# kenziyuliu/ChineseCheckersAgent

Hardware: AMD Instinct MI355X
Metric: mcts_node_expansions_per_s (self-play with the policy/value net, 4096 games x 400 sims/move per GPU); BASELINE games/s = config.games_per_s: selfplay() calls that RETURNED per second, discarded ones included (train.py:61-64 counts them); config.games_won_per_s: those that returned a history (higher is better)
Workload: dtype f32

## Files before the change

### chinesecheckersagent_amd/csrc/ccsp_net.hip

```cpp
#include <cmath>
#include <cstring>
#include <type_traits>
#include <vector>
#include "ccsp_common.h"

namespace {

typedef float f32x4 __attribute__((ext_vector_type(4)));

#ifndef CCSP_NET_LDX
#define CCSP_NET_LDX 68
#define CCSP_NET_LDY 36
#endif
constexpr int LDX = CCSP_NET_LDX;
constexpr int LDY = CCSP_NET_LDY;
constexpr int LDI = 12;
constexpr int NPOL = 294, NPOL_PAD = 304;
#ifndef CCSP_NET_LDS_BIAS_ALL
#define CCSP_NET_LDS_BIAS_ALL 0
#endif
#ifndef CCSP_NET_PDG
#define CCSP_NET_PDG 1
#endif
#ifndef CCSP_NET_SEG_STEM
#define CCSP_NET_SEG_STEM 1
#endif
#ifndef CCSP_NET_SEG_L1
#define CCSP_NET_SEG_L1 1
#endif
#ifndef CCSP_NET_SEG_L2
#define CCSP_NET_SEG_L2 4
#endif
#ifndef CCSP_NET_SEG_L3
#define CCSP_NET_SEG_L3 1
#endif
#ifndef CCSP_NET_SEG_PC
#define CCSP_NET_SEG_PC 1
#endif

struct Layout {
    int trunk_b;
    int stem_w, stem_b;
    int l1_w[9], l1_b[9], l2_w[9], l2_b[9], l3_w[9], l3_b[9];
    int pc_w, pc_b, pf_w, pf_b;
    int vc_w, vc_b, f1_w, f1_b, f2_w, f2_b;
    int total;
};

constexpr Layout make_layout() {
    Layout L{};
    int o = 0;
    auto take = [&](int n) { int r = o; o += (n + 3) & ~3; return r; };
    L.trunk_b = take(64 + 9 * 128 + 16);
    L.stem_w = take(4 * 5 * 256); L.stem_b = L.trunk_b;
    for (int i = 0; i < 9; i++) {
        L.l1_w[i] = take(2 * 4 * 256); L.l1_b[i] = L.trunk_b + 64 + i * 128;
        L.l2_w[i] = take(2 * 18 * 256); L.l2_b[i] = L.trunk_b + 64 + i * 128 + 32;
        L.l3_w[i] = take(4 * 2 * 256); L.l3_b[i] = L.trunk_b + 64 + i * 128 + 64;
    }
    L.pc_w = take(1 * 4 * 256); L.pc_b = L.trunk_b + 64 + 9 * 128;
    L.pf_w = take(5 * 100 * 256); L.pf_b = take(NPOL_PAD);
    L.vc_w = take(64); L.vc_b = take(1);
    L.f1_w = take(25 * 32); L.f1_b = take(32);
    L.f2_w = take(32); L.f2_b = take(1);
    L.total = o;
    return L;
}
constexpr Layout LAY = make_layout();
constexpr int BLK_STRIDE = LAY.l1_w[1] - LAY.l1_w[0];
constexpr bool layout_is_regular() {
    for (int i = 0; i < 9; i++)
        if (LAY.l1_w[i] != LAY.l1_w[0] + i * BLK_STRIDE || LAY.l2_w[i] != LAY.l2_w[0] + i * BLK_STRIDE || LAY.l3_w[i] != LAY.l3_w[0] + i * BLK_STRIDE) return false;
    return true;
}
static_assert(layout_is_regular(), "the blocks' weights are BLK_STRIDE floats apart");
constexpr int BIAS_STEM = 0, BIAS_BLK = 64, BIAS_PER_BLK = 128, BIAS_L1 = 0, BIAS_L2 = 32, BIAS_L3 = 64, BIAS_PC = BIAS_BLK + 9 * BIAS_PER_BLK, BIAS_N = BIAS_PC + 16;
static_assert(LAY.stem_b == LAY.trunk_b + BIAS_STEM && LAY.l1_b[3] == LAY.trunk_b + BIAS_BLK + 3 * BIAS_PER_BLK + BIAS_L1 && LAY.l2_b[8] == LAY.trunk_b + BIAS_BLK + 8 * BIAS_PER_BLK + BIAS_L2 &&
              LAY.l3_b[0] == LAY.trunk_b + BIAS_BLK + BIAS_L3 && LAY.pc_b == LAY.trunk_b + BIAS_PC && BIAS_N % 4 == 0 && LAY.trunk_b % 4 == 0, "Smem::bias is the blob's trunk_b region");

constexpr int PLAIN_TOTAL = 4032 + 64 + 9 * (2048 + 32 + 9216 + 32 + 2048 + 64) + 1024 + 16 + 117600 + 294 + 64 + 1 + 800 + 32 + 32 + 1;
static_assert(PLAIN_TOTAL == 244920, "249852 parameters minus the 4 x 1233 BatchNorm values folded away");

constexpr int PAD0 = 7, PADPOS = 36;
#ifndef CCSP_NET_SKIP_DEAD_TAPS
#define CCSP_NET_SKIP_DEAD_TAPS 1
#endif
#ifndef CCSP_NET_KB_FENCE
#define CCSP_NET_KB_FENCE 1
#endif
#ifndef CCSP_NET_CM4
#define CCSP_NET_CM4 1
#endif
constexpr unsigned char CELL8[25] = {0, 1, 2, 3, 6, 7,   4, 9, 14, 19, 11, 12,   24, 23, 22, 21, 16, 17,   20, 15, 10, 5, 8, 13,   18};
constexpr unsigned char CELL4[25] = {0, 1, 2, 3,  4, 9, 14, 19,  6, 7, 8, 11,   24, 23, 22, 21,  20, 15, 10, 5,  12, 13, 16, 17,   18};
constexpr int on_edge(int cell, int e) { return e == 0 ? cell / 5 == 0 : (e == 1 ? cell % 5 == 4 : (e == 2 ? cell / 5 == 4 : cell % 5 == 0)); }
constexpr bool interior(int cell) { return !on_edge(cell, 0) && !on_edge(cell, 1) && !on_edge(cell, 2) && !on_edge(cell, 3); }
constexpr bool cells_ok() {
    bool seen8[25] = {}, seen4[25] = {};
    for (int i = 0; i < 25; i++) {
        if (CELL8[i] > 24 || seen8[CELL8[i]] || CELL4[i] > 24 || seen4[CELL4[i]]) return false;
        seen8[CELL8[i]] = true; seen4[CELL4[i]] = true;
    }
    for (int g = 0; g < 4; g++)
        for (int i = 0; i < 6; i++)
            if (i < 4 ? !on_edge(CELL8[6 * g + i], g) : !interior(CELL8[6 * g + i])) return false;
    for (int g = 0; g < 2; g++)
        for (int i = 0; i < 12; i++)
            if (i < 8 ? !on_edge(CELL4[12 * g + i], 2 * g + i / 4) : !interior(CELL4[12 * g + i])) return false;
    return interior(CELL8[24]) && interior(CELL4[24]);
}
static_assert(cells_ok(), "CELL8 / CELL4: permutations; the edge tiles on their edges, the other tiles interior");
template <int NB>
constexpr unsigned long long cell_pack(int from) {
    unsigned long long v = 0;
    for (int i = 0; i < 12 && from + i < 25; i++) v |= (unsigned long long)(NB == 8 ? CELL8 : CELL4)[from + i] << (5 * i);
    return v;
}
template <int NB>
__device__ __forceinline__ int cell_of(int idx) {
    const unsigned long long w = idx < 12 ? cell_pack<NB>(0) : (idx < 24 ? cell_pack<NB>(12) : cell_pack<NB>(24));
    return (int)((w >> (5 * (idx < 12 ? idx : (idx < 24 ? idx - 12 : 0)))) & 31);
}
constexpr unsigned EDGE_DEAD[4] = {0x0003Fu , 0x30C30u , 0x3F000u , 0x030C3u };
constexpr int CM_PAD = 3, CM_SLOTS = 35;

template <int NBv, int NWv>
struct Cfg {
    static constexpr int NB = NBv, NW = NWv, NTH = NWv * 64, ROWS = NBv * 25, MT = (NBv * 25 + 15) / 16;
    static constexpr int NSPLIT = NWv / 2;
    static constexpr bool ALLSPLIT = MT < NSPLIT;
    static constexpr int NSH = ALLSPLIT ? NSPLIT / MT : NSPLIT;
    static constexpr int XTILES = ALLSPLIT ? MT : 1;
    static constexpr int F32 = MT / NSPLIT;
    static constexpr int F32A = F32 > 0 ? F32 : 1;
    static constexpr int XT = ALLSPLIT ? 0 : MT - F32 * NSPLIT;
    static constexpr int NH = NWv / 4;
    static constexpr int F64 = (MT + NH - 1) / NH;
    static constexpr int M64 = NH == 2 ? F64 : 0;
    static constexpr int F64B = NH == 2 ? MT - F64 : F64;
    static constexpr bool PADFULL = F32 * NSPLIT * 16 > ROWS;
    static constexpr int HB = NBv < 4 ? 4 : NBv;
    static constexpr int NSEG = CCSP_NET_SEG_L2;
    static constexpr bool CELLMAJOR = (NBv == 8 || (NBv == 4 && CCSP_NET_CM4)) && CCSP_NET_SKIP_DEAD_TAPS;
    static constexpr int NE = CELLMAJOR ? 2 : 0;
    static constexpr unsigned dead_of(int g, int slot) { return NBv == 8 ? EDGE_DEAD[g] : EDGE_DEAD[2 * g + slot]; }
    static constexpr int xseg_of(int g) { return NBv == 8 ? (g == 2 ? 3 : (g == 3 ? 2 : g)) : g; }
    static constexpr int PADROWS_ = CELLMAJOR ? CM_SLOTS * NBv : PAD0 + NBv * PADPOS + 1, PADROWS_HEADS = (HB * 400 + LDY - 1) / LDY;
    static constexpr int PADROWS = PADROWS_ > PADROWS_HEADS ? PADROWS_ : PADROWS_HEADS;
    static constexpr int INROWS = NBv * 49 + 56;
    static constexpr int NTW = (19 + NWv - 1) / NWv;
#ifndef CCSP_NET_PDG_SMALL
#define CCSP_NET_PDG_SMALL 1
#endif
    static constexpr int PDG = NBv <= 2 ? CCSP_NET_PDG_SMALL : CCSP_NET_PDG;
    static_assert((XT == 0 || XT == 1) && (F32 >= 1 || ALLSPLIT) && F32 <= 3 && F64 <= 7 && MT <= 13 && (NWv == 4 || NWv == 8), "tile shares");
    static_assert(!ALLSPLIT || (NSPLIT % MT == 0 && NSEG % NSH == 0 && F64 == 1 && F64B == 1 && M64 + 1 == MT), "<1, 8>: two waves per 3x3 tile job, one 64-column job per wave");
};

template <typename C>
struct Smem {
    float y1[C::PADROWS * LDY];
    static constexpr int Y2A = C::MT * 16 * LDY, Y2B = C::INROWS * LDI, Y2C = 256 + C::HB * (NPOL_PAD + 32);
    static constexpr int Y2N = Y2A > Y2B ? (Y2A > Y2C ? Y2A : Y2C) : (Y2B > Y2C ? Y2B : Y2C);
    float y2[Y2N];
    float x[C::MT * 16 * LDX > 4 * C::HB * 320 ? C::MT * 16 * LDX : 4 * C::HB * 320];
    float part[2 * C::XTILES][C::NSEG][256];
    float bias[(C::NB < 8 || CCSP_NET_LDS_BIAS_ALL) ? BIAS_N : 4];
    static_assert(C::INROWS * LDI <= Y2N, "the staged input planes alias y2");
    static_assert(C::MT * 16 * 16 <= C::PADROWS * LDY && C::HB * 400 <= C::PADROWS * LDY, "the policy conv output aliases y1");
    static_assert(256 + C::HB * (NPOL_PAD + 32) <= Y2N, "logits and value scratch alias y2");
};
#ifndef CCSP_NET_NO_LDS_ASSERT
static_assert(sizeof(Smem<Cfg<8, 8>>) + 3 * 6900 <= 160 * 1024, "<8,8>: one evaluator workgroup per CU plus three tree-kernel workgroups");
#endif
static_assert(sizeof(Smem<Cfg<4, 4>>) + 3 * 6900 <= 160 * 1024, "<4,4>: an evaluator workgroup per CU plus three tree-kernel workgroups (two per CU no longer fit: the shape carries batches of at most one workgroup per CU)");
static_assert(sizeof(Smem<Cfg<2, 8>>) <= 64 * 1024, "<2,8>: a small workgroup");
static_assert(sizeof(Smem<Cfg<1, 8>>) <= 64 * 1024, "<1,8>: a small workgroup");

typedef __attribute__((address_space(3))) float lds_float;
typedef __attribute__((address_space(3))) f32x4 lds_f32x4;
__device__ __forceinline__ lds_float *lds_opaque(float *p) {
    unsigned a = (unsigned)(size_t)(lds_float *)p;
    asm volatile("" : "+v"(a));
    return (lds_float *)(size_t)a;
}
__device__ __forceinline__ f32x4 lds_load4(const lds_float *p, int off) { return *reinterpret_cast<const lds_f32x4 *>(p + off); }
__device__ __forceinline__ void lds_store4(lds_float *p, int off, const f32x4 &v) { *reinterpret_cast<lds_f32x4 *>(p + off) = v; }

struct WBuf {
    __amdgpu_buffer_rsrc_t r;
    int voff;
    __device__ __forceinline__ f32x4 load(int float_off) const {
        typedef int i32x4 __attribute__((ext_vector_type(4)));
        return __builtin_bit_cast(f32x4, __builtin_amdgcn_raw_buffer_load_b128(r, voff, float_off * 4, 0));
    }
};

__device__ __forceinline__ f32x4 mfma4(const f32x4 a, const f32x4 b, f32x4 c) {
    c = __builtin_amdgcn_mfma_f32_16x16x4f32(a[0], b[0], c, 0, 0, 0);
    c = __builtin_amdgcn_mfma_f32_16x16x4f32(a[1], b[1], c, 0, 0, 0);
    c = __builtin_amdgcn_mfma_f32_16x16x4f32(a[2], b[2], c, 0, 0, 0);
    c = __builtin_amdgcn_mfma_f32_16x16x4f32(a[3], b[3], c, 0, 0, 0);
    return c;
}

#ifndef CCSP_NET_NPRE
#define CCSP_NET_NPRE 3
#endif
constexpr int NPREMAX = CCSP_NET_NPRE;
template <int KB> struct Pre { static constexpr int N = KB < NPREMAX ? KB : NPREMAX; };
template <int KBN>
__device__ __forceinline__ void prefetch(const WBuf &wb, int wbase, int nt, f32x4 (&pre)[NPREMAX]) {
#pragma unroll
    for (int d = 0; d < Pre<KBN>::N; d++) pre[d] = wb.load(wbase + nt * KBN * 256 + d * 256);
}

template <int KB, int NSEG>
__device__ __forceinline__ constexpr int seg_of(int kb) {
    int seg = 0;
    for (int c = 1; c < NSEG; c++) seg += kb >= (KB * c) / NSEG ? 1 : 0;
    return seg;
}
template <int NMT, int KB, int NSEG, typename AFrag, typename Next, typename Epi>
__device__ __forceinline__ void gemm_tiles(const WBuf &wb, int wbase, int nt, int mt0, f32x4 (&pre)[NPREMAX], AFrag afrag, Next next, Epi epi) {
    constexpr int NPRE = Pre<KB>::N;
    constexpr int PB = NPRE + 1 < KB ? NPRE + 1 : KB;
    static_assert(NSEG >= 1 && NSEG <= KB, "a segment is at least one k-block");
    f32x4 acc[NMT][NSEG];
#pragma unroll
    for (int i = 0; i < NMT; i++)
#pragma unroll
        for (int c = 0; c < NSEG; c++) acc[i][c] = f32x4{0.f, 0.f, 0.f, 0.f};
    const int w0 = wbase + nt * KB * 256;
    f32x4 bq[PB];
#pragma unroll
    for (int d = 0; d < NPRE; d++) bq[d] = pre[d];
    f32x4 a[2][NMT];
// ... 214 lines not shown
        for (int c = 1; c < SPW; c++) seg += j >= seg_lo(c) ? 1 : 0;
        if (j + 1 < KBP) a[(j + 1) & 1] = afrag(kb0 + j + 1);
        const f32x4 b = bq[j];
#pragma unroll
        for (int q = 0; q < 4; q++) accx[seg] = __builtin_amdgcn_mfma_f32_16x16x4f32(b[q], a[j & 1][q], accx[seg], 0, 0, 0);
    }
#pragma unroll
    for (int c = 0; c < SPW; c++) lds_store4(part, c * 256, accx[c]);
}

template <int NMT, int KB, int NSPLIT, int NSEG, int MINE_C, typename AFrag, typename Next, typename Epi, typename EpiX>
__device__ __forceinline__ void gemm_tiles_last(const WBuf &wb, int wbase, int nt, int mt0, int xmt, int kpart, f32x4 (&pre)[NPREMAX],
                                                AFrag afrag, Next next, Epi epi, EpiX epix) {
    constexpr int NPRE = Pre<KB>::N;
    constexpr int PB = NPRE + 1 < KB ? NPRE + 1 : KB;
    static_assert(NSEG >= 1 && NSEG <= KB, "a segment is at least one k-block");
    const bool mine = MINE_C < 0 ? kpart == NSPLIT - 1 : MINE_C != 0;
    f32x4 acc[NMT + 1][NSEG];
#pragma unroll
    for (int i = 0; i <= NMT; i++)
#pragma unroll
        for (int c = 0; c < NSEG; c++) acc[i][c] = f32x4{0.f, 0.f, 0.f, 0.f};
    const int w0 = wbase + nt * KB * 256;
    f32x4 bq[PB];
#pragma unroll
    for (int d = 0; d < NPRE; d++) bq[d] = pre[d];
    f32x4 a[2][NMT + 1];
#pragma unroll
    for (int i = 0; i < NMT; i++) a[0][i] = afrag(mt0 + i, 0, i);
    if (MINE_C != 0) a[0][NMT] = afrag(xmt, 0, NMT);
#pragma unroll
    for (int kb = 0; kb < KB; kb++) {
        int seg = 0;
#pragma unroll
        for (int c = 1; c < NSEG; c++) seg += kb >= (KB * c) / NSEG ? 1 : 0;
        if (kb + 1 < KB) {
#pragma unroll
            for (int i = 0; i < NMT; i++) a[(kb + 1) & 1][i] = afrag(mt0 + i, kb + 1, i);
            if (MINE_C != 0) a[(kb + 1) & 1][NMT] = afrag(xmt, kb + 1, NMT);
        }
        if (kb + PB - 1 < KB && kb + PB - 1 >= NPRE) bq[(kb + PB - 1) % PB] = wb.load(w0 + (kb + PB - 1) * 256);
        const f32x4 b = bq[kb % PB];
#pragma unroll
        for (int j = 0; j < 4; j++) {
#pragma unroll
            for (int i = 0; i < NMT; i++)
                acc[i][seg] = __builtin_amdgcn_mfma_f32_16x16x4f32(b[j], a[kb & 1][i][j], acc[i][seg], 0, 0, 0);
            if (MINE_C > 0) acc[NMT][seg] = __builtin_amdgcn_mfma_f32_16x16x4f32(b[j], a[kb & 1][NMT][j], acc[NMT][seg], 0, 0, 0);
        }
        if (MINE_C < 0 && mine) {
#pragma unroll
            for (int j = 0; j < 4; j++)
                acc[NMT][seg] = __builtin_amdgcn_mfma_f32_16x16x4f32(b[j], a[kb & 1][NMT][j], acc[NMT][seg], 0, 0, 0);
        }
    }
    next();
#pragma unroll
    for (int i = 0; i <= NMT; i++) {
        f32x4 sum = acc[i][0];
#pragma unroll
        for (int c = 1; c < NSEG; c++) sum = sum + acc[i][c];
        if (i < NMT) epi(mt0 + i, sum, i);
        else if (mine) epix(sum);
    }
}

__device__ __forceinline__ float relu(float v) { return __builtin_amdgcn_fmed3f(v, 0.0f, __builtin_inff()); }

template <typename F>
__device__ __forceinline__ void for_each_out(int mt, const f32x4 &acc, F f) {
    const int lane = threadIdx.x & 63;
    const int col = lane & 15, r0 = mt * 16 + 4 * (lane >> 4);
#pragma unroll
    for (int reg = 0; reg < 4; reg++) f(r0 + reg, col, acc[reg]);
}

#ifdef CCSP_STAMPS
__device__ unsigned long long net_stamps[64];
__device__ unsigned long long net_stamps2[8][8];
#define NET_STAMP(i) do { if (blockIdx.x == 0 && threadIdx.x == 0) net_stamps[i] = __builtin_amdgcn_s_memtime(); } while (0)
#define NET_STAMP2(pt) do { if (blockIdx.x == 0 && lane == 0 && blk == 4) net_stamps2[wave][pt] = __builtin_amdgcn_s_memtime(); } while (0)
__device__ unsigned long long net_stamps3[8][8];
#define NET_STAMP3(pt) do { if (blockIdx.x == 0 && lane == 0 && blk == 4) net_stamps3[wave][pt] = __builtin_amdgcn_s_memtime(); } while (0)
#else
#define NET_STAMP(i) do { } while (0)
#define NET_STAMP2(pt) do { } while (0)
#define NET_STAMP3(pt) do { } while (0)
#endif

template <typename C, bool REQ>
__global__ __launch_bounds__(C::NTH) void net_forward_kernel(const float *__restrict__ W, const float *__restrict__ planes, int n,
                                                             float *__restrict__ logits_out, double *__restrict__ p_out,
                                                             float *__restrict__ v_out, const uint16_t *__restrict__ moves) {
    constexpr int NB = C::NB, NTH = C::NTH, ROWS = C::ROWS, MT = C::MT, NSPLIT = C::NSPLIT, PADROWS = C::PADROWS, INROWS = C::INROWS,
                  NW = C::NW, F32 = C::F32, F32A = C::F32A, F64 = C::F64, F64B = C::F64B, M64 = C::M64, XT = C::XT, HB = C::HB;
    constexpr bool AS = C::ALLSPLIT;
    extern __shared__ __attribute__((aligned(16))) unsigned char smem_raw[];
    Smem<C> &S = *reinterpret_cast<Smem<C> *>(smem_raw);
    const int tid = threadIdx.x, lane = tid & 63;
    const int wave = __builtin_amdgcn_readfirstlane(tid >> 6);
    const int q = lane >> 4, l15 = lane & 15;
    const long long s0 = (long long)blockIdx.x * NB;
    const int here = (int)((n - s0) < NB ? (n - s0) : NB);

    WBuf wb;
    wb.r = __builtin_amdgcn_make_buffer_rsrc(const_cast<float *>(W), 0, LAY.total * 4, 0x00020000);
    wb.voff = lane * 16;

#ifdef CCSP_STAMPS
    if (blockIdx.x == 0 && threadIdx.x == 0) net_stamps[62] = __builtin_amdgcn_s_memtime();
#endif
    float *in = S.y2;
    static_assert((PADROWS * LDY) % 4 == 0, "y1 is cleared 16 bytes at a time");
    for (int i = tid * 4; i < PADROWS * LDY; i += NTH * 4) *reinterpret_cast<f32x4 *>(&S.y1[i]) = f32x4{0.f, 0.f, 0.f, 0.f};
    if constexpr (NB < 8 || CCSP_NET_LDS_BIAS_ALL)
    for (int i = tid; i < BIAS_N / 4; i += NTH)
        *reinterpret_cast<f32x4 *>(&S.bias[4 * i]) = *reinterpret_cast<const f32x4 *>(W + LAY.trunk_b + 4 * i);
    const ccsp_request *rq = reinterpret_cast<const ccsp_request *>(planes) + s0;
    if constexpr (REQ) {
        static_assert((INROWS * LDI) % 4 == 0, "the staging area is cleared 16 bytes at a time");
        for (int i = tid * 4; i < INROWS * LDI; i += NTH * 4) *reinterpret_cast<f32x4 *>(&in[i]) = f32x4{0.f, 0.f, 0.f, 0.f};
        __syncthreads();
        struct PlaneWriter {
            float *base;
            struct Ref { float *p; __device__ __forceinline__ void operator=(uint8_t val) const { *p = (float)val; } };
            __device__ __forceinline__ Ref operator[](int i) const { const int cell = i / 7; return Ref{base + cell * LDI + (i - 7 * cell)}; }
        };
        for (int t = tid; t < here * 12; t += NTH) {
            const int s = t / 12, k = t - 12 * s;
            if (rq[s].kind == 0) continue;
            const ccsp_sr st = ccsp_load_sr(&rq[s].state);
            ccsp_scatter_checker(st, (int)rq[s].player, k, PlaneWriter{in + s * 49 * LDI});
        }
        for (int t = tid; t < here * 49; t += NTH) {
            const int s = t / 49, cell = t - 49 * s;
            if (rq[s].kind != 0 && rq[s].player == 2) in[(s * 49 + cell) * LDI + 6] = 1.0f;
        }
    } else if constexpr ((NB * 343) % 4 != 0) {
        for (int i = tid; i < INROWS * LDI; i += NTH) {
            const int cellg = i / LDI, ch = i % LDI, s = cellg / 49, cell = cellg % 49;
            in[i] = (ch < 7 && s < here) ? planes[(s0 + s) * 343 + cell * 7 + ch] : 0.0f;
        }
    } else {
        constexpr int NV = (NB * 343) / 4, PER = (NV + NTH - 1) / NTH;
        const f32x4 *src = reinterpret_cast<const f32x4 *>(planes + s0 * 343);
        const int nreal = here * 343;
        f32x4 v[PER];
#pragma unroll
        for (int r = 0; r < PER; r++) {
            const int e = (tid + r * NTH) * 4;
            v[r] = f32x4{0.f, 0.f, 0.f, 0.f};
            if (e + 3 < nreal) v[r] = src[tid + r * NTH];
            else if (e < nreal) { for (int j = 0; j < 4; j++) if (e + j < nreal) v[r][j] = planes[s0 * 343 + e + j]; }
        }
        static_assert((INROWS * LDI) % 4 == 0, "the staging area is cleared 16 bytes at a time");
        for (int i = tid * 4; i < INROWS * LDI; i += NTH * 4) *reinterpret_cast<f32x4 *>(&in[i]) = f32x4{0.f, 0.f, 0.f, 0.f};
        __syncthreads();
#pragma unroll
        for (int r = 0; r < PER; r++) {
            const int e = (tid + r * NTH) * 4;
#pragma unroll
            for (int j = 0; j < 4; j++) {
                const unsigned ee = (unsigned)(e + j);
                if ((int)ee < nreal) {
                    const unsigned cellg = __umulhi(ee, 613566757u);
                    in[cellg * LDI + (ee - 7u * cellg)] = v[r][j];
                }
            }
        }
    }
#ifdef CCSP_EXP_NET_INPUT_DELAY
// ... 159 lines not shown
                    auto run = [&](auto G) {
                        constexpr int g = decltype(G)::value;
                        if constexpr (TAIL4) {
                            gemm_tiles_split<F32A, 18, C::NSEG, NSPLIT, C::NE, true, C::dead_of(g, 0), C::dead_of(g, 1), -1>(wb, (LAY.l2_w[0] + wo), nt2, mt3, MT - 1, 0, pre, afrag, next, epi, partw);
                            if constexpr (g < 2) {
                                auto afrag4 = [&](int kb, int q4) -> f32x4 {
                                    const int tap = kb >> 1;
                                    return lds_load4(ytail, ((tap / 3) * 6 + tap % 3) * TAPROW + (kb & 1) * 16 + 4 * q4);
                                };
                                auto job = [&](auto SEG) {
                                    constexpr int seg = decltype(SEG)::value, kb0 = (18 * seg) / C::NSEG, kb1 = (18 * (seg + 1)) / C::NSEG;
                                    const f32x4 t = tail_tile_4x4<kb0, kb1 - kb0>(wbt, (LAY.l2_w[0] + wo), afrag4);
#pragma unroll
                                    for (int r = 0; r < 4; r++) partt[seg * 256 + r * 4] = t[r];
                                };
                                if (nt2 == 0) job(std::integral_constant<int, 2 * g>{});
                                else job(std::integral_constant<int, 2 * g + 1>{});
                            }
                        } else
                        gemm_tiles_split<F32A, 18, C::NSEG, NSPLIT, C::NE, true, C::dead_of(g, 0), C::dead_of(g, 1), C::xseg_of(g)>(wb, (LAY.l2_w[0] + wo), nt2, mt3, MT - 1, 0, pre, afrag, next, epi, partw);
                    };
                    if (qr == 0) run(std::integral_constant<int, 0>{});
                    else if (NSPLIT == 2 || qr == 1) run(std::integral_constant<int, 1>{});
                    else if (qr == 2) run(std::integral_constant<int, NSPLIT == 2 ? 1 : 2>{});
                    else run(std::integral_constant<int, NSPLIT == 2 ? 1 : 3>{});
                } else
                    gemm_tiles_split<F32A, 18, C::NSEG, NSPLIT, 0, false, 0u, 0u, 0>(wb, (LAY.l2_w[0] + wo), nt2, mt3, MT - 1, kshare, pre, afrag, next, epi, partw);
            }
            NET_STAMP(32 + blk);
#ifdef CCSP_STAMPS
            if (blockIdx.x == 0 && lane == 0 && blk == 4) {
                net_stamps[44 + wave] = __builtin_amdgcn_s_memtime();
                net_stamps[52 + wave] = __builtin_amdgcn_s_getreg(4 | (0 << 6) | (31 << 11));
            }
#endif
        }
        __syncthreads();
        NET_STAMP(3 + 3 * blk);
        {
            const int nt = wave & 3, half = wave >> 2, mt0 = half * M64;
            NET_STAMP2(0);
            const bool has_x = AS || (XT && half == C::NH - 1);
            constexpr int XSLOT = F64B - 1;
            const int xt = AS ? mt0 : 0;
            f32x4 ax[2];
            if (has_x) {
#pragma unroll
                for (int kb = 0; kb < 2; kb++) {
                    f32x4 v = lds_load4(partr, kb * C::NSEG * 256);
#pragma unroll
                    for (int c = 1; c < C::NSEG; c++) v = v + lds_load4(partr, (kb * C::NSEG + c) * 256);
                    ax[kb] = relu4(v + bias4(bb + BIAS_L2 + kb * 16));
                }
            }
            auto afrag = [&](int mt, int kb, int i) -> f32x4 {
                if (i == XSLOT && has_x) return ax[kb];
                return lds_load4(y2r, i * 16 * LDY + kb * 16);
            };
            const f32x4 bv = bias4(bb + BIAS_L3 + nt * 16);
            auto epi = [&](int mt, const f32x4 &acc, int i) {
                xr[i] = relu4(acc + bv + xr[i]);
                lds_store4(xown, i * 16 * LDX, xr[i]);
            };
            NET_STAMP2(1);
            auto next = [&]() {
                NET_STAMP2(2);
                prefetch<4>(wb, blk < 8 ? LAY.l1_w[0] + wo + BLK_STRIDE : LAY.pc_w, blk < 8 ? nt2 : 0, pre);
            };
            if constexpr (GROUPS) {
                static_assert(!GROUPS || XSLOT >= group1(F64B), "the tile fed from Smem::part is in the last group");
                if (half == 0) gemm_tiles_grouped<F64, group1(F64), 2>(wb, (LAY.l3_w[0] + wo), nt, mt0, pre, afrag, next, epi);
                else gemm_tiles_grouped<F64B, group1(F64B), 2>(wb, (LAY.l3_w[0] + wo), nt, mt0, pre, afrag, next, epi);
            } else
            if (F64B == F64 || half == 0) gemm_tiles<F64, 2, CCSP_NET_SEG_L3>(wb, (LAY.l3_w[0] + wo), nt, mt0, pre, afrag, next, epi);
            else gemm_tiles<F64B, 2, CCSP_NET_SEG_L3>(wb, (LAY.l3_w[0] + wo), nt, mt0, pre, afrag, next, epi);
            NET_STAMP2(3);
        }
        __syncthreads();
        NET_STAMP2(4);
        NET_STAMP(4 + 3 * blk);
    }

    float *pc = S.y1;
    {
        const int mt0 = 2 * wave < MT - 2 ? 2 * wave : MT - 2;
        const lds_float *const xpc = lds_opaque(&S.x[(mt0 * 16 + l15) * LDX + 4 * q]);
        auto afrag = [&](int, int kb, int i) -> f32x4 { return lds_load4(xpc, i * 16 * LDX + kb * 16); };
        const f32x4 bv = bias4(BIAS_PC);
        int pcat[2];
#pragma unroll
        for (int i = 0; i < 2; i++) {
            const int row = (mt0 + i) * 16 + l15;
            int s, pos;
            row_sp(row, s, pos);
            pcat[i] = (CM ? (row < ROWS ? s * 25 + pos : row) : row) * 16 + 4 * q;
        }
        auto epi = [&](int, const f32x4 &acc, int i) {
            *reinterpret_cast<f32x4 *>(&pc[pcat[i]]) = relu4(acc + bv);
        };
        gemm_tiles<2, 4, CCSP_NET_SEG_PC>(wb, LAY.pc_w, 0, mt0, pre, afrag, []() {}, epi);
    }
    float *vc = S.y2;
    float *lg = S.y2 + 256;
    if (tid < ROWS) {
        const float *wv = W + LAY.vc_w;
        float acc = W[LAY.vc_b];
        const float *xr = &S.x[tid * LDX];
#pragma unroll 8
        for (int k = 0; k < 64; k++) acc += xr[k] * wv[k];
        int s, pos;
        row_sp(tid, s, pos);
        vc[CM ? s * 25 + pos : tid] = acc > 0.f ? acc : 0.f;
    }
    __syncthreads();
    NET_STAMP(29);

    float *part = S.x;
    {
        constexpr int GPQ = 25, NHALF = NW / 4, TPW = (5 + NHALF - 1) / NHALF, PG = HB / 4, PDG = C::PDG;
        const int kq = wave & 3, th = wave >> 2;
        int woff[TPW];
        bool valid[TPW];
#pragma unroll
        for (int t = 0; t < TPW; t++) {
            const int T = th * TPW + t;
            valid[t] = T < 5;
            woff[t] = LAY.pf_w + ((valid[t] ? T : 0) * 100 + kq * GPQ) * 256;
        }
        f32x4 acc[TPW][PG], bq[PDG + 1][TPW];
#pragma unroll
        for (int t = 0; t < TPW; t++)
#pragma unroll
            for (int g = 0; g < PG; g++) acc[t][g] = f32x4{0.f, 0.f, 0.f, 0.f};
#pragma unroll
        for (int d = 0; d < PDG; d++)
#pragma unroll
            for (int t = 0; t < TPW; t++) bq[d][t] = wb.load(woff[t] + d * 256);
        const float *arow = &pc[(lane & 3) * 400 + kq * GPQ * 4];
        f32x4 a[2][PG];
#pragma unroll
        for (int g = 0; g < PG; g++) a[0][g] = *reinterpret_cast<const f32x4 *>(arow + g * 1600);
#pragma unroll
        for (int kg = 0; kg < GPQ; kg++) {
            if (kg + 1 < GPQ) {
#pragma unroll
                for (int g = 0; g < PG; g++) a[(kg + 1) & 1][g] = *reinterpret_cast<const f32x4 *>(arow + g * 1600 + (kg + 1) * 4);
            }
            if (kg + PDG < GPQ) {
#pragma unroll
                for (int t = 0; t < TPW; t++) bq[(kg + PDG) % (PDG + 1)][t] = wb.load(woff[t] + (kg + PDG) * 256);
            }
#pragma unroll
            for (int t = 0; t < TPW; t++) {
                if (t + 1 < TPW || valid[t]) {
#pragma unroll
                    for (int j = 0; j < 4; j++)
#pragma unroll
                        for (int g = 0; g < PG; g++)
                            acc[t][g] = __builtin_amdgcn_mfma_f32_4x4x1f32(a[kg & 1][g][j], bq[kg % (PDG + 1)][t][j], acc[t][g], 0, 0, 0);
                }
            }
        }
#pragma unroll
        for (int t = 0; t < TPW; t++) {
            if (valid[t]) {
                const int T = th * TPW + t;
#pragma unroll
                for (int g = 0; g < PG; g++)
#pragma unroll
                    for (int r = 0; r < 4; r++) part[(kq * HB + 4 * g + r) * 320 + T * 64 + lane] = acc[t][g][r];
            }
        }
    }
    __syncthreads();
    for (int i = tid; i < NB * NPOL; i += NTH) {
        const int s = i / NPOL, col = i - s * NPOL;
        const float q0 = part[(0 * HB + s) * 320 + col], q1 = part[(1 * HB + s) * 320 + col], q2 = part[(2 * HB + s) * 320 + col],
                    q3 = part[(3 * HB + s) * 320 + col];
        lg[s * NPOL_PAD + col] = ((q0 + q1) + q2) + q3 + W[LAY.pf_b + col];
    }
    float *h1 = S.y2 + 256 + NB * NPOL_PAD;
    if (tid < NB * 32) {
        const int s = tid >> 5, u = tid & 31;
        const float *w1 = W + LAY.f1_w;
        float acc = W[LAY.f1_b + u];
#pragma unroll 5
        for (int i = 0; i < 25; i++) acc += vc[s * 25 + i] * w1[i * 32 + u];
        h1[s * 32 + u] = acc > 0.f ? acc : 0.f;
    }
    __syncthreads();
    NET_STAMP(30);
    if (tid < here) {
        const float *w2 = W + LAY.f2_w;
        float acc = W[LAY.f2_b];
        for (int u = 0; u < 32; u++) acc += h1[tid * 32 + u] * w2[u];
        if (!REQ || rq[tid].kind != 0) v_out[s0 + tid] = tanhf(acc);
    }
    for (int s = wave; s < here; s += NTH / 64) {
        const float *row = lg + s * NPOL_PAD;
        float mx = -INFINITY;
        for (int i = lane; i < NPOL; i += 64) mx = fmaxf(mx, row[i]);
        for (int m = 32; m >= 1; m >>= 1) mx = fmaxf(mx, __shfl_xor(mx, m));
        double e[5];
        double sum = 0.0;
#pragma unroll
        for (int j = 0; j < 5; j++) {
            const int i = lane + 64 * j;
            e[j] = i < NPOL ? exp((double)row[i] - (double)mx) : 0.0;
            sum += e[j];
        }
        for (int m = 32; m >= 1; m >>= 1) sum += __shfl_xor(sum, m);
        if constexpr (REQ) {
            double *pd = reinterpret_cast<double *>(S.x) + wave * 296;
            if (rq[s].kind != 0) {
#pragma unroll
                for (int j = 0; j < 5; j++) {
                    const int i = lane + 64 * j;
                    if (i < NPOL) pd[i] = e[j] / sum;
                }
                __builtin_amdgcn_wave_barrier();
                const int k = (int)rq[s].k < CCSP_MAX_MOVES ? (int)rq[s].k : CCSP_MAX_MOVES;
                const uint16_t *mrow = moves + (s0 + s) * CCSP_REQUEST_MOVES;
#pragma unroll
                for (int h = 0; h < 2; h++) {
                    const int j = lane + 64 * h;
                    if (j < k) { const int a = mrow[j] & 0x1FF; p_out[(s0 + s) * CCSP_REQUEST_MOVES + j] = a < NPOL ? pd[a] : 0.0; }
                }
                __builtin_amdgcn_wave_barrier();
            }
        } else {
#pragma unroll
        for (int j = 0; j < 5; j++) {
            const int i = lane + 64 * j;
            if (i < NPOL) {
                if (p_out) p_out[(s0 + s) * NPOL + i] = e[j] / sum;
                if (logits_out) logits_out[(s0 + s) * NPOL + i] = row[i];
            }
        }
        }
    }
    NET_STAMP(31);
#ifdef CCSP_STAMPS
    if (blockIdx.x == 0 && threadIdx.x == 0) net_stamps[61] = __builtin_amdgcn_s_memrealtime();
#endif
}

void pack_gemm(const std::vector<float> &Wkn, int K, int N, int KB, int NT, float *out) {
    for (int nt = 0; nt < NT; nt++)
        for (int kb = 0; kb < KB; kb++)
            for (int lane = 0; lane < 64; lane++)
                for (int j = 0; j < 4; j++) {
                    const int k = 16 * kb + 4 * (lane >> 4) + j, nn = 16 * nt + (lane & 15);
                    out[((nt * KB + kb) * 64 + lane) * 4 + j] = (k < K && nn < N) ? Wkn[(size_t)k * N + nn] : 0.0f;
                }
}

}

template <typename C, bool REQ = false>
static int launch_net(const float *packed, const float *planes, int n, float *logits, double *p, float *v, void *stream, bool *attr_set,
                      const uint16_t *moves = nullptr) {
    int dev = 0;
    CCSP_HIPCHK(hipGetDevice(&dev));
    if (dev < 0 || dev >= 64 || !attr_set[dev]) {
        CCSP_HIPCHK(hipFuncSetAttribute(reinterpret_cast<const void *>(net_forward_kernel<C, REQ>),
                                        hipFuncAttributeMaxDynamicSharedMemorySize, (int)sizeof(Smem<C>)));
        if (dev >= 0 && dev < 64) attr_set[dev] = true;
    }
    const int grid = (n + C::NB - 1) / C::NB;
    hipLaunchKernelGGL((net_forward_kernel<C, REQ>), dim3(grid), dim3(C::NTH), sizeof(Smem<C>), (hipStream_t)stream, packed, planes, n, logits, p, v, moves);
    CCSP_HIPCHK(hipGetLastError());
    return CCSP_OK;
}

static int g_net_shape = 0;
#ifndef CCSP_NET_SMALL
#define CCSP_NET_SMALL 1024
#define CCSP_NET_TINY 512
#endif
#ifndef CCSP_NET_ONE
#define CCSP_NET_ONE 256
#endif
static int pick_shape(int n) { return n <= CCSP_NET_ONE ? 1 : (n <= CCSP_NET_TINY ? 2 : (n <= CCSP_NET_SMALL ? 4 : 8)); }

extern "C" {

int ccsp_net_plain_size(void) { return PLAIN_TOTAL; }
int ccsp_net_packed_size(void) { return LAY.total; }

int ccsp_net_pack(const float *plain, float *packed) {
    if (!plain || !packed) return CCSP_EINVAL;
    memset(packed, 0, sizeof(float) * (size_t)LAY.total);
    const float *p = plain;
    {
        std::vector<float> Wkn(80 * 64, 0.0f);
        for (int tap = 0; tap < 9; tap++)
            for (int ch = 0; ch < 7; ch++)
                for (int o = 0; o < 64; o++) Wkn[(size_t)(tap * 8 + ch) * 64 + o] = p[(tap * 7 + ch) * 64 + o];
        pack_gemm(Wkn, 80, 64, 5, 4, packed + LAY.stem_w);
        p += 4032;
        memcpy(packed + LAY.stem_b, p, 64 * sizeof(float)); p += 64;
    }
    for (int b = 0; b < 9; b++) {
        { std::vector<float> Wkn(p, p + 64 * 32); pack_gemm(Wkn, 64, 32, 4, 2, packed + LAY.l1_w[b]); p += 2048; }
        memcpy(packed + LAY.l1_b[b], p, 32 * sizeof(float)); p += 32;
        { std::vector<float> Wkn(p, p + 288 * 32); pack_gemm(Wkn, 288, 32, 18, 2, packed + LAY.l2_w[b]); p += 9216; }
        memcpy(packed + LAY.l2_b[b], p, 32 * sizeof(float)); p += 32;
        { std::vector<float> Wkn(p, p + 32 * 64); pack_gemm(Wkn, 32, 64, 2, 4, packed + LAY.l3_w[b]); p += 2048; }
        memcpy(packed + LAY.l3_b[b], p, 64 * sizeof(float)); p += 64;
    }
    { std::vector<float> Wkn(p, p + 64 * 16); pack_gemm(Wkn, 64, 16, 4, 1, packed + LAY.pc_w); p += 1024; }
    memcpy(packed + LAY.pc_b, p, 16 * sizeof(float)); p += 16;
    for (int T = 0; T < 5; T++)
        for (int g = 0; g < 100; g++)
            for (int lane = 0; lane < 64; lane++)
                for (int j = 0; j < 4; j++) {
                    const int k = 4 * g + j, col = 64 * T + lane;
                    packed[LAY.pf_w + ((T * 100 + g) * 64 + lane) * 4 + j] = col < 294 ? p[(size_t)k * 294 + col] : 0.0f;
                }
    p += 117600;
    memcpy(packed + LAY.pf_b, p, 294 * sizeof(float)); p += 294;
    memcpy(packed + LAY.vc_w, p, 64 * sizeof(float)); p += 64;
    packed[LAY.vc_b] = *p; p += 1;
    memcpy(packed + LAY.f1_w, p, 800 * sizeof(float)); p += 800;
    memcpy(packed + LAY.f1_b, p, 32 * sizeof(float)); p += 32;
    memcpy(packed + LAY.f2_w, p, 32 * sizeof(float)); p += 32;
    packed[LAY.f2_b] = *p; p += 1;
    return (p - plain) == PLAIN_TOTAL ? CCSP_OK : CCSP_EINVAL;
}

int ccsp_debug_net_shape(int positions_per_workgroup) {
    g_net_shape = (positions_per_workgroup == 1 || positions_per_workgroup == 2 || positions_per_workgroup == 4 || positions_per_workgroup == 8) ? positions_per_workgroup : 0;
    return g_net_shape;
}

int ccsp_net_forward(const float *packed, const float *planes, int n, float *logits, double *p, float *v, void *stream) {
    if (n < 0 || (n > 0 && (!packed || !planes || !v))) return CCSP_EINVAL;
    if (n == 0) return CCSP_OK;
    static bool attr8[64] = {false}, attr4[64] = {false}, attr2[64] = {false}, attr1[64] = {false};
    const int shape = g_net_shape ? g_net_shape : pick_shape(n);
    if (shape == 1) return launch_net<Cfg<1, 8>>(packed, planes, n, logits, p, v, stream, attr1);
    if (shape == 2) return launch_net<Cfg<2, 8>>(packed, planes, n, logits, p, v, stream, attr2);
    if (shape == 4) return launch_net<Cfg<4, 4>>(packed, planes, n, logits, p, v, stream, attr4);
    return launch_net<Cfg<8, 8>>(packed, planes, n, logits, p, v, stream, attr8);
}

int ccsp_net_forward_requests(const float *packed, const ccsp_request *req, const uint16_t *moves, int n, double *pk, float *v, void *stream) {
    if (n < 0 || (n > 0 && (!packed || !req || !moves || !pk || !v))) return CCSP_EINVAL;
    if (n == 0) return CCSP_OK;
    static bool attr8[64] = {false}, attr4[64] = {false}, attr2[64] = {false}, attr1[64] = {false};
    const float *in = reinterpret_cast<const float *>(req);
    const int shape = g_net_shape ? g_net_shape : pick_shape(n);
    if (shape == 1) return launch_net<Cfg<1, 8>, true>(packed, in, n, nullptr, pk, v, stream, attr1, moves);
    if (shape == 2) return launch_net<Cfg<2, 8>, true>(packed, in, n, nullptr, pk, v, stream, attr2, moves);
    if (shape == 4) return launch_net<Cfg<4, 4>, true>(packed, in, n, nullptr, pk, v, stream, attr4, moves);
    return launch_net<Cfg<8, 8>, true>(packed, in, n, nullptr, pk, v, stream, attr8, moves);
}

#ifdef CCSP_STAMPS
int ccsp_debug_net_stamps(unsigned long long *out) {
    const bool more = out[63] == 0x5eedULL;
    const bool more3 = more && out[62] == 0x5eedULL;
    CCSP_HIPCHK(hipMemcpyFromSymbol(out, HIP_SYMBOL(net_stamps), 64 * sizeof(unsigned long long)));
    if (more) CCSP_HIPCHK(hipMemcpyFromSymbol(out + 64, HIP_SYMBOL(net_stamps2), 64 * sizeof(unsigned long long)));
    if (more3) CCSP_HIPCHK(hipMemcpyFromSymbol(out + 128, HIP_SYMBOL(net_stamps3), 64 * sizeof(unsigned long long)));
    return CCSP_OK;
}
#endif

}
```

Before: 23.73 million.

## Prefetch policy-dense weights during policy conv and trim head tail work

For the 8-sample shape, the first few policy-dense weight groups are now loaded during the policy conv GEMM so they are already in registers when the dense stage starts. The prefetch depth for this shape goes from 1 to 3. The dense loop is specialized per tile half to the number of live column tiles, and scheduling fences are placed between k-groups. The first value-head dense layer moves ahead of the barrier with a full unroll, so it overlaps other waves' policy work. In exchange, register pressure rises from the larger prefetch ring, and debug stamp hooks are added.

```diff
diff --git a/chinesecheckersagent_amd/csrc/ccsp_net.hip b/chinesecheckersagent_amd/csrc/ccsp_net.hip
--- a/chinesecheckersagent_amd/csrc/ccsp_net.hip
+++ b/chinesecheckersagent_amd/csrc/ccsp_net.hip
@@ -21,6 +21,18 @@
 #endif
 #ifndef CCSP_NET_PDG
 #define CCSP_NET_PDG 1
+#endif
+#ifndef CCSP_NET_DENSE_EARLY
+#define CCSP_NET_DENSE_EARLY 1
+#endif
+#ifndef CCSP_NET_DENSE_LIVE
+#define CCSP_NET_DENSE_LIVE 1
+#endif
+#ifndef CCSP_NET_VAL2_EARLY
+#define CCSP_NET_VAL2_EARLY 1
+#endif
+#ifndef CCSP_NET_PD_FENCE
+#define CCSP_NET_PD_FENCE 1
 #endif
 #ifndef CCSP_NET_SEG_STEM
 #define CCSP_NET_SEG_STEM 1
@@ -152,7 +164,14 @@
 #ifndef CCSP_NET_PDG_SMALL
 #define CCSP_NET_PDG_SMALL 1
 #endif
-    static constexpr int PDG = NBv <= 2 ? CCSP_NET_PDG_SMALL : CCSP_NET_PDG;
+#ifndef CCSP_NET_PDG_LARGE
+#define CCSP_NET_PDG_LARGE 3
+#endif
+    static constexpr int PDG = NBv <= 2 ? CCSP_NET_PDG_SMALL : (NBv == 8 ? CCSP_NET_PDG_LARGE : CCSP_NET_PDG);
+    static constexpr bool DENSE_EARLY = NBv == 8 && CCSP_NET_DENSE_EARLY;
+    static constexpr bool DENSE_LIVE = NBv == 8 && CCSP_NET_DENSE_LIVE && (DENSE_EARLY || PDG > 1);
+    static constexpr bool VAL2_EARLY = NBv == 8 && CCSP_NET_VAL2_EARLY && (DENSE_EARLY || PDG > 1);
+    static constexpr bool PD_FENCE = NBv == 8 && CCSP_NET_PD_FENCE && (DENSE_EARLY || PDG > 1);
     static_assert((XT == 0 || XT == 1) && (F32 >= 1 || ALLSPLIT) && F32 <= 3 && F64 <= 7 && MT <= 13 && (NWv == 4 || NWv == 8), "tile shares");
     static_assert(!ALLSPLIT || (NSPLIT % MT == 0 && NSEG % NSH == 0 && F64 == 1 && F64B == 1 && M64 + 1 == MT), "<1, 8>: two waves per 3x3 tile job, one 64-column job per wave");
 };
@@ -533,11 +552,26 @@
 #define NET_STAMP2(pt) do { if (blockIdx.x == 0 && lane == 0 && blk == 4) net_stamps2[wave][pt] = __builtin_amdgcn_s_memtime(); } while (0)
 __device__ unsigned long long net_stamps3[8][8];
 #define NET_STAMP3(pt) do { if (blockIdx.x == 0 && lane == 0 && blk == 4) net_stamps3[wave][pt] = __builtin_amdgcn_s_memtime(); } while (0)
+__device__ unsigned long long net_stamps4[8][8];
+#define NET_STAMP4(pt) do { if (blockIdx.x == 0 && lane == 0) net_stamps4[wave][pt] = __builtin_amdgcn_s_memtime(); } while (0)
 #else
 #define NET_STAMP(i) do { } while (0)
 #define NET_STAMP2(pt) do { } while (0)
 #define NET_STAMP3(pt) do { } while (0)
-#endif
+#define NET_STAMP4(pt) do { } while (0)
+#endif
+
+template <int NB, int UNR>
+__device__ __forceinline__ void value_dense1(const float *__restrict__ W, const float *vc, float *h1, int tid) {
+    if (tid < NB * 32) {
+        const int s = tid >> 5, u = tid & 31;
+        const float *w1 = W + LAY.f1_w;
+        float acc = W[LAY.f1_b + u];
+#pragma unroll UNR
+        for (int i = 0; i < 25; i++) acc += vc[s * 25 + i] * w1[i * 32 + u];
+        h1[s * 32 + u] = acc > 0.f ? acc : 0.f;
+    }
+}
 
 template <typename C, bool REQ>
 __global__ __launch_bounds__(C::NTH) void net_forward_kernel(const float *__restrict__ W, const float *__restrict__ planes, int n,
@@ -863,6 +897,8 @@
     }
 
     float *pc = S.y1;
+    constexpr int EPDG = C::DENSE_EARLY ? C::PDG : 1, ETPW = (5 + NW / 4 - 1) / (NW / 4);
+    f32x4 bqe[EPDG][ETPW];
     {
         const int mt0 = 2 * wave < MT - 2 ? 2 * wave : MT - 2;
         const lds_float *const xpc = lds_opaque(&S.x[(mt0 * 16 + l15) * LDX + 4 * q]);
@@ -879,8 +915,19 @@
         auto epi = [&](int, const f32x4 &acc, int i) {
             *reinterpret_cast<f32x4 *>(&pc[pcat[i]]) = relu4(acc + bv);
         };
+        if constexpr (C::DENSE_EARLY) {
+            auto next = [&]() {
+                const int T0 = (wave >> 2) * ETPW;
+#pragma unroll
+                for (int d = 0; d < EPDG; d++)
+#pragma unroll
+                    for (int t = 0; t < ETPW; t++) bqe[d][t] = wb.load(LAY.pf_w + ((T0 + t < 5 ? T0 + t : 0) * 100 + (wave & 3) * 25 + d) * 256);
+            };
+            gemm_tiles<2, 4, CCSP_NET_SEG_PC>(wb, LAY.pc_w, 0, mt0, pre, afrag, next, epi);
+        } else
         gemm_tiles<2, 4, CCSP_NET_SEG_PC>(wb, LAY.pc_w, 0, mt0, pre, afrag, []() {}, epi);
     }
+    NET_STAMP(41);
     float *vc = S.y2;
     float *lg = S.y2 + 256;
     if (tid < ROWS) {
@@ -913,16 +960,50 @@
         for (int t = 0; t < TPW; t++)
 #pragma unroll
             for (int g = 0; g < PG; g++) acc[t][g] = f32x4{0.f, 0.f, 0.f, 0.f};
+        static_assert(!C::DENSE_EARLY || (EPDG == PDG && ETPW == TPW), "the groups requested behind the policy conv are the ring's first PDG");
 #pragma unroll
         for (int d = 0; d < PDG; d++)
 #pragma unroll
-            for (int t = 0; t < TPW; t++) bq[d][t] = wb.load(woff[t] + d * 256);
+            for (int t = 0; t < TPW; t++) {
+                if constexpr (C::DENSE_EARLY) bq[d][t] = bqe[d][t];
+                else bq[d][t] = wb.load(woff[t] + d * 256);
+            }
         const float *arow = &pc[(lane & 3) * 400 + kq * GPQ * 4];
         f32x4 a[2][PG];
 #pragma unroll
         for (int g = 0; g < PG; g++) a[0][g] = *reinterpret_cast<const f32x4 *>(arow + g * 1600);
+        NET_STAMP(42);
+        NET_STAMP4(0);
+        if constexpr (C::DENSE_LIVE) {
+            static_assert(TPW < 5 && 2 * TPW >= 5, "two tile halves: TPW column tiles and 5 - TPW");
+            auto groups = [&](auto live) {
+                constexpr int NT = decltype(live)::value;
+#pragma unroll
+                for (int kg = 0; kg < GPQ; kg++) {
+                    if constexpr (C::PD_FENCE) __builtin_amdgcn_sched_barrier(0);
+                    if (kg + 1 < GPQ) {
+#pragma unroll
+                        for (int g = 0; g < PG; g++) a[(kg + 1) & 1][g] = *reinterpret_cast<const f32x4 *>(arow + g * 1600 + (kg + 1) * 4);
+                    }
+                    if (kg + PDG < GPQ) {
+#pragma unroll
+                        for (int t = 0; t < NT; t++) bq[(kg + PDG) % (PDG + 1)][t] = wb.load(woff[t] + (kg + PDG) * 256);
+                    }
+#pragma unroll
+                    for (int t = 0; t < NT; t++)
+#pragma unroll
+                        for (int j = 0; j < 4; j++)
+#pragma unroll
+                            for (int g = 0; g < PG; g++)
+                                acc[t][g] = __builtin_amdgcn_mfma_f32_4x4x1f32(a[kg & 1][g][j], bq[kg % (PDG + 1)][t][j], acc[t][g], 0, 0, 0);
+                }
+            };
+            if (th == 0) groups(std::integral_constant<int, TPW>{});
+            else groups(std::integral_constant<int, 5 - TPW>{});
+        } else {
 #pragma unroll
         for (int kg = 0; kg < GPQ; kg++) {
+            if constexpr (C::PD_FENCE) __builtin_amdgcn_sched_barrier(0);
             if (kg + 1 < GPQ) {
 #pragma unroll
                 for (int g = 0; g < PG; g++) a[(kg + 1) & 1][g] = *reinterpret_cast<const f32x4 *>(arow + g * 1600 + (kg + 1) * 4);
@@ -942,6 +1023,9 @@
                 }
             }
         }
+        }
+        NET_STAMP(43);
+        NET_STAMP4(1);
 #pragma unroll
         for (int t = 0; t < TPW; t++) {
             if (valid[t]) {
@@ -953,22 +1037,21 @@
             }
         }
     }
+    if constexpr (C::VAL2_EARLY) value_dense1<NB, 25>(W, vc, S.y2 + 256 + NB * NPOL_PAD, tid);
+    NET_STAMP4(2);
     __syncthreads();
+    NET_STAMP4(3);
     for (int i = tid; i < NB * NPOL; i += NTH) {
         const int s = i / NPOL, col = i - s * NPOL;
         const float q0 = part[(0 * HB + s) * 320 + col], q1 = part[(1 * HB + s) * 320 + col], q2 = part[(2 * HB + s) * 320 + col],
                     q3 = part[(3 * HB + s) * 320 + col];
         lg[s * NPOL_PAD + col] = ((q0 + q1) + q2) + q3 + W[LAY.pf_b + col];
     }
+    NET_STAMP(63);
+    NET_STAMP4(4);
     float *h1 = S.y2 + 256 + NB * NPOL_PAD;
-    if (tid < NB * 32) {
-        const int s = tid >> 5, u = tid & 31;
-        const float *w1 = W + LAY.f1_w;
-        float acc = W[LAY.f1_b + u];
-#pragma unroll 5
-        for (int i = 0; i < 25; i++) acc += vc[s * 25 + i] * w1[i * 32 + u];
-        h1[s * 32 + u] = acc > 0.f ? acc : 0.f;
-    }
+    if constexpr (!C::VAL2_EARLY) value_dense1<NB, 5>(W, vc, h1, tid);
+    NET_STAMP4(5);
     __syncthreads();
     NET_STAMP(30);
     if (tid < here) {
@@ -1021,6 +1104,7 @@
         }
     }
     NET_STAMP(31);
+    NET_STAMP4(6);
 #ifdef CCSP_STAMPS
     if (blockIdx.x == 0 && threadIdx.x == 0) net_stamps[61] = __builtin_amdgcn_s_memrealtime();
 #endif
@@ -1147,6 +1231,10 @@
     if (more3) CCSP_HIPCHK(hipMemcpyFromSymbol(out + 128, HIP_SYMBOL(net_stamps3), 64 * sizeof(unsigned long long)));
     return CCSP_OK;
 }
-#endif
-
-}
+int ccsp_debug_net_stamps_heads(unsigned long long *out) {
+    CCSP_HIPCHK(hipMemcpyFromSymbol(out, HIP_SYMBOL(net_stamps4), 64 * sizeof(unsigned long long)));
+    return CCSP_OK;
+}
+#endif
+
+}
```

Result: no change. 23.95 million (median of 6 runs) (+1.0%).
